# wangys16/FreeSplat

Measured on AMD Instinct MI355X. Metric: rendered views/sec @ 968x1296, 1.0M Gaussians, higher is better.
Workload: dtype f32

## Files before the change

freesplat_amd/csrc/raster_fwd.hip:

```cpp
#include <stdlib.h>

#include <type_traits>

#include "fs_common.h"

namespace fs {

template <int M>
__device__ __forceinline__ uint32_t lane_xor(uint32_t v)
{
    if constexpr (M == 1) return (uint32_t)__builtin_amdgcn_mov_dpp((int)v, 0xB1, 0xF, 0xF, true);
    else if constexpr (M == 2) return (uint32_t)__builtin_amdgcn_mov_dpp((int)v, 0x4E, 0xF, 0xF, true);
    else if constexpr (M == 3) return (uint32_t)__builtin_amdgcn_mov_dpp((int)v, 0x1B, 0xF, 0xF, true);
    else if constexpr (M < 32) return (uint32_t)__builtin_amdgcn_ds_swizzle((int)v, (M << 10) | 0x1F);
    else return (uint32_t)__shfl_xor((int)v, M, 64);
}
template <int M>
__device__ __forceinline__ unsigned long long lane_xor64(unsigned long long v)
{
    const uint32_t lo = lane_xor<M>((uint32_t)v), hi = lane_xor<M>((uint32_t)(v >> 32));
    return ((unsigned long long)hi << 32) | lo;
}

template <int DEG>
__device__ __forceinline__ void eval_sh(const float* __restrict__ sh, float3 dir, float* rgb,
                                        uint8_t& clampbits, int cs, int ks)
{
    float b[16];
    sh_basis<DEG>(dir.x, dir.y, dir.z, b);
    constexpr int NB = (DEG + 1) * (DEG + 1);
    clampbits = 0;
#pragma unroll
    for (int c = 0; c < 3; ++c) {
        const float* s = sh + c * cs;
        float acc = b[0] * s[0];
#pragma unroll
        for (int k = 1; k < NB; ++k) acc = acc + b[k] * s[k * ks];
        acc = acc + 0.5f;
        if (acc < 0.0f) clampbits |= (uint8_t)(1u << c);
        rgb[c] = fmaxf(acc, 0.0f);
    }
}

__device__ __forceinline__ void stage_rows(float* lds, const float* __restrict__ src, size_t base,
                                           int cnt, int per)
{
    const float* s = src + base * per;
    const int total = cnt * per;
    if ((((uintptr_t)s) & 15) == 0) {
        const int nv = total >> 2;
        int k = threadIdx.x;
        for (; k + 768 < nv; k += 1024) {
            const float4 v0 = ((const float4*)s)[k], v1 = ((const float4*)s)[k + 256];
            const float4 v2 = ((const float4*)s)[k + 512], v3 = ((const float4*)s)[k + 768];
            ((float4*)lds)[k] = v0; ((float4*)lds)[k + 256] = v1;
            ((float4*)lds)[k + 512] = v2; ((float4*)lds)[k + 768] = v3;
        }
        for (; k < nv; k += 256) ((float4*)lds)[k] = ((const float4*)s)[k];
        for (int k = (nv << 2) + threadIdx.x; k < total; k += blockDim.x) lds[k] = s[k];
    } else {
        for (int k = threadIdx.x; k < total; k += blockDim.x) lds[k] = s[k];
    }
}



struct QuadForm {
    float a, b, c;
    float Q;
    float D;
    float vplus;
    float Vmax;
    float inv2a;
};
__device__ __forceinline__ QuadForm quad_form(const float4 r0, const float4 r1)
{
    QuadForm f;
    f.a = -r0.z; f.c = -r0.w; f.b = -r1.x;
    f.Q = -(r1.z - 1e-3f * (1.0f + fabsf(r1.z)));
    f.D = 4.0f * f.a * f.c - f.b * f.b;
    const float invD = __builtin_amdgcn_rcpf(f.D);
    const float U = __builtin_amdgcn_sqrtf(fmaxf(4.0f * f.c * f.Q * invD, 0.0f));
    f.vplus = -f.b * __builtin_amdgcn_rcpf(2.0f * f.c) * U;
    f.Vmax = __builtin_amdgcn_sqrtf(fmaxf(4.0f * f.a * f.Q * invD, 0.0f));
    f.inv2a = __builtin_amdgcn_rcpf(2.0f * f.a);
    return f;
}
struct Band { float uL, uR; };
constexpr float kEps = 2e-5f;
__device__ __forceinline__ Band band_interval(const QuadForm& f, float vlo, float vhi)
{
    Band o;
    if (f.Q < 0.0f || vlo > f.Vmax + kEps || vhi < -f.Vmax - kEps) { o.uL = 3.0e38f; o.uR = -3.0e38f; return o; }
    const float vr = fminf(vhi, fmaxf(vlo, f.vplus)), vl = fminf(vhi, fmaxf(vlo, -f.vplus));
    const float sr = __builtin_amdgcn_sqrtf(fmaxf(4.0f * f.a * f.Q - f.D * vr * vr, 0.0f));
    const float sl = __builtin_amdgcn_sqrtf(fmaxf(4.0f * f.a * f.Q - f.D * vl * vl, 0.0f));
    o.uR = (-f.b * vr + sr) * f.inv2a;
    o.uL = (-f.b * vl - sl) * f.inv2a;
    const float w = kEps * (1.0f + fabsf(o.uR) + fabsf(o.uL));
    o.uR += w; o.uL -= w;
    return o;
}
struct RowBands { Band top, bot; };
__device__ __forceinline__ RowBands row_bands(const QuadForm& f, const float4 r0, int ty)
{
    const float v0 = (float)(ty * kTile) - r0.y;
    RowBands r;
    r.top = band_interval(f, v0, v0 + 7.0f);
    r.bot = band_interval(f, v0 + 8.0f, v0 + 15.0f);
    return r;
}
__device__ __forceinline__ uint32_t quad_mask_row(const RowBands& rb, const float4 r0, int tx)
{
    const float u0 = (float)(tx * kTile) - r0.x, u1 = u0 + 8.0f;
    uint32_t m = 0;
    if (!(u0 > rb.top.uR) && !(u0 + 7.0f < rb.top.uL)) m |= 1u;
    if (!(u1 > rb.top.uR) && !(u1 + 7.0f < rb.top.uL)) m |= 2u;
    if (!(u0 > rb.bot.uR) && !(u0 + 7.0f < rb.bot.uL)) m |= 4u;
    if (!(u1 > rb.bot.uR) && !(u1 + 7.0f < rb.bot.uL)) m |= 8u;
    return m;
}

__device__ __forceinline__ uint32_t band_cells(const Band& b, float px, int cell0, int ncell)
{
    const uint32_t full = ncell >= 32 ? 0xFFFFFFFFu : ((1u << ncell) - 1u);
    if (b.uL > b.uR) return 0u;
    if (!(b.uL <= b.uR)) return full;
    const float lo_f = ceilf((b.uL + px - 7.0f) * 0.125f - 1e-3f), hi_f = floorf((b.uR + px) * 0.125f + 1e-3f);
    const int lo = max((int)lo_f, cell0) - cell0, hi = min((int)hi_f, cell0 + ncell - 1) - cell0;
    if (lo > hi) return 0u;
    return ((2u << hi) - (1u << lo)) & full;
}
__device__ __forceinline__ unsigned long long pack_quad_masks(const QuadForm& f, const float4 r0, ushort4 rc)
{
    unsigned long long m = 0;
    const int rw = rc.z - rc.x, cell0 = 2 * rc.x, ncell = 2 * rw;
    int k = 0;
    for (int y = rc.y; y < rc.w; ++y) {
        const RowBands rb = row_bands(f, r0, y);
        const uint32_t top = band_cells(rb.top, r0.x, cell0, ncell), bot = band_cells(rb.bot, r0.x, cell0, ncell);
        for (int x = 0; x < rw; ++x, ++k) {
            const uint32_t nib = ((top >> (2 * x)) & 3u) | (((bot >> (2 * x)) & 3u) << 2);
            m |= (unsigned long long)nib << (4 * k);
        }
    }
    return m;
}

__device__ __forceinline__ uint32_t spread2(uint32_t x)
{
    x = (x | (x << 4)) & 0x0F0Fu;
    return (x | (x << 2)) & 0x3333u;
}
__device__ __forceinline__ unsigned long long pack_quad_masks4(const QuadForm& f, const float4 r0, ushort4 rc, bool cull, uint32_t& nz)
{
    unsigned long long m = 0;
    const int rw = rc.z - rc.x, rh = rc.w - rc.y, cell0 = 2 * rc.x, ncell = 2 * rw;
    const uint32_t rowfull = (1u << rw) - 1u;
    nz = 0u;
#pragma unroll
    for (int r = 0; r < 4; ++r) {
        if (r < rh) {
            const RowBands rb = row_bands(f, r0, rc.y + r);
            const uint32_t top = band_cells(rb.top, r0.x, cell0, ncell), bot = band_cells(rb.bot, r0.x, cell0, ncell);
            m |= (unsigned long long)(spread2(top) | (spread2(bot) << 2)) << (16 * r);
            uint32_t any = top | bot;
            any = (any | (any >> 1)) & 0x55u;
            any = (any | (any >> 1)) & 0x33u;
            any = (any | (any >> 2)) & 0x0Fu;
            nz |= (cull ? any : rowfull) << (4 * r);
        }
    }
    return m;
}

__device__ __forceinline__ void stage_rows_half(float* lds, const _Float16* __restrict__ src, size_t base, int cnt,
                                                int per)
{
    const _Float16* s = src + base * per;
    const int total = cnt * per;
    typedef _Float16 half8 __attribute__((ext_vector_type(8)));
    int done = 0;
    if ((((uintptr_t)s) & 15) == 0) {
        const int nv = total >> 3;
        auto put = [&](int k, const half8 v) {
            ((float4*)lds)[2 * k] = make_float4((float)v[0], (float)v[1], (float)v[2], (float)v[3]);
            ((float4*)lds)[2 * k + 1] = make_float4((float)v[4], (float)v[5], (float)v[6], (float)v[7]);
        };
        int k = threadIdx.x;
        for (; k + 256 < nv; k += 512) {
            const half8 v0 = ((const half8*)s)[k], v1 = ((const half8*)s)[k + 256];
            put(k, v0); put(k + 256, v1);
        }
        for (; k < nv; k += 256) put(k, ((const half8*)s)[k]);
        done = nv << 3;
    }
    for (int k = done + threadIdx.x; k < total; k += blockDim.x) lds[k] = (float)s[k];
}

struct Projected {
    float4 r0, r1, r2;
    ushort4 rect;
    uint8_t cb;
    int rad;
};
__device__ __forceinline__ Projected project_gaussian(
    const fs_raster_dims& d, bool live, float3 p_in, const float (&c_in)[6], float op, size_t i,
    const float* __restrict__ colors, const float* sh , int sh_cs, int sh_ks,
    const float* __restrict__ view, const float* __restrict__ proj, const float* __restrict__ campos,
    float tanfovx, float tanfovy, bool rescale, float wscale)
{
    Projected o;
    o.r0 = make_float4(0, 0, 0, 0); o.r1 = o.r0; o.r2 = o.r0;
    o.rect = make_ushort4(0, 0, 0, 0);
    o.cb = 0;
    o.rad = 0;
    float3 p = p_in;
    if (rescale) { p.x = p.x * wscale; p.y = p.y * wscale; p.z = p.z * wscale; }
    const float3 pv = xform43(view, p);
    if (live && pv.z > 0.2f) {
        const float4 ph = xform44(proj, p);
        const float pw = 1.0f / (ph.w + 0.0000001f);
        const float ndcx = ph.x * pw, ndcy = ph.y * pw;
        const float fx = (float)d.W / (2.0f * tanfovx), fy = (float)d.H / (2.0f * tanfovy);
        float c3[6];
#pragma unroll
        for (int k = 0; k < 6; ++k) c3[k] = c_in[k];
        if (rescale) {
            const float s2 = wscale * wscale;
#pragma unroll
            for (int k = 0; k < 6; ++k) c3[k] = c3[k] * s2;
        }
        const Cov2D cv = project_cov(view, p, c3, fx, fy, tanfovx, tanfovy);
        const float det = cv.a * cv.c - cv.b * cv.b;
        if (det != 0.0f) {
            const float det_inv = 1.0f / det;
            const float cA = cv.c * det_inv, cB = -cv.b * det_inv, cC = cv.a * det_inv;
            const float mid = 0.5f * (cv.a + cv.c);
            const float sq = sqrtf(fmaxf(0.1f, mid * mid - det));
            const float l1 = mid + sq, l2 = mid - sq;
            const float my_radius = ceilf(3.0f * sqrtf(fmaxf(l1, l2)));
            const float px = ((ndcx + 1.0f) * (float)d.W - 1.0f) * 0.5f;
            const float py = ((ndcy + 1.0f) * (float)d.H - 1.0f) * 0.5f;
            const int r = (int)my_radius;
            const int gx = (d.W + kTile - 1) / kTile, gy = (d.H + kTile - 1) / kTile;
            const int x0 = min(gx, max(0, (int)((px - (float)r) / (float)kTile)));
            const int y0 = min(gy, max(0, (int)((py - (float)r) / (float)kTile)));
            const int x1 = min(gx, max(0, (int)((px + (float)r + (float)(kTile - 1)) / (float)kTile)));
            const int y1 = min(gy, max(0, (int)((py + (float)r + (float)(kTile - 1)) / (float)kTile)));
            if ((x1 - x0) * (y1 - y0) > 0) {
                float rgb[3];
                if (colors) {
                    rgb[0] = colors[3 * i];
                    rgb[1] = colors[3 * i + 1];
                    rgb[2] = colors[3 * i + 2];
                } else {
                    float3 dir = make_float3(p.x - campos[0], p.y - campos[1], p.z - campos[2]);
                    const float len = sqrtf(dir.x * dir.x + dir.y * dir.y + dir.z * dir.z);
                    dir.x = dir.x / len; dir.y = dir.y / len; dir.z = dir.z / len;
                    switch (d.sh_degree) {
                        case 0: eval_sh<0>(sh, dir, rgb, o.cb, sh_cs, sh_ks); break;
                        case 1: eval_sh<1>(sh, dir, rgb, o.cb, sh_cs, sh_ks); break;
                        case 2: eval_sh<2>(sh, dir, rgb, o.cb, sh_cs, sh_ks); break;
                        default: eval_sh<3>(sh, dir, rgb, o.cb, sh_cs, sh_ks); break;
                    }
                }
                float thr;
                if (op > 0.0f) {
                    const float l = -logf(255.0f * op);
                    thr = l - (0.001f + 1e-5f * fabsf(l));
                } else {
                    thr = 1.0f;
                }
                o.r0 = make_float4(px, py, -0.5f * cA, -0.5f * cC);
                o.r1 = make_float4(-cB, op, thr, pv.z);
                o.r2 = make_float4(rgb[0], rgb[1], rgb[2], 0.0f);
                o.rect = make_ushort4((unsigned short)x0, (unsigned short)y0, (unsigned short)x1,
                                      (unsigned short)y1);
                o.rad = r;
            }
        }
    }
    return o;
}

template <bool SR>
__device__ __forceinline__ void load_mean_cov(const fs_raster_dims& d, const float* __restrict__ means3D,
                                              const float* __restrict__ cov3D, size_t i, float3& p_in, float (&c_in)[6])
{
    p_in = make_float3(means3D[3 * i], means3D[3 * i + 1], means3D[3 * i + 2]);
    if constexpr (SR) {
        float row[7];
#pragma unroll
        for (int k = 0; k < 7; ++k) row[k] = cov3D[7 * i + k];
        cov_from_scale_rot(row, c_in);
    } else if (d.flags & FS_RASTER_COV_FULL) {
        const float* cr = cov3D + 9 * i;
        c_in[0] = cr[0]; c_in[1] = cr[1]; c_in[2] = cr[2]; c_in[3] = cr[4]; c_in[4] = cr[5]; c_in[5] = cr[8];
    } else {
#pragma unroll
        for (int k = 0; k < 6; ++k) c_in[k] = cov3D[6 * i + k];
    }
}

constexpr int kWaveBins = 512;

__device__ __forceinline__ void bin_wave(const fs_raster_dims& d, int lane, uint32_t* s_cnt, uint32_t i, const Projected& pr,
                                         uint32_t* __restrict__ tile_counts, unsigned long long* __restrict__ keys,
                                         uint32_t tile_cap)
{
    const float4 r0 = pr.r0, r1 = pr.r1;
    const ushort4 rect = pr.rect;
    const bool valid = pr.rad > 0;
    const bool cull = (d.flags & FS_RASTER_TILE_CULL) != 0;
    const int gx = (d.W + kTile - 1) / kTile;
    const QuadForm qf = quad_form(r0, r1);
    const int rw = rect.z - rect.x, rh = rect.w - rect.y;
    const int area = rw * rh;
    const bool small = area <= 16;
    const bool all4 = __builtin_amdgcn_ballot_w64(valid && (rw > 4 || rh > 4)) == 0ull;
    unsigned long long qm = 0;
    uint32_t nz = 0u;
    if (all4) { if (valid) qm = pack_quad_masks4(qf, r0, rect, cull, nz); }
    else if (valid && small) qm = pack_quad_masks(qf, r0, rect);
    const unsigned long long key_hi = ((unsigned long long)__float_as_uint(r1.w) << 32) | (i << 4);
    int x0 = valid ? (int)rect.x : 0x7fff, y0 = valid ? (int)rect.y : 0x7fff;
    int x1 = valid ? (int)rect.z : 0, y1 = valid ? (int)rect.w : 0;
#define FS_BOX_STEP(M)                                                                                           \
    {                                                                                                            \
        const int lo = (int)lane_xor<M>((uint32_t)((x0 << 16) | y0)), hi = (int)lane_xor<M>((uint32_t)((x1 << 16) | y1)); \
        x0 = min(x0, lo >> 16); y0 = min(y0, lo & 0xffff);                                                       \
        x1 = max(x1, hi >> 16); y1 = max(y1, hi & 0xffff);                                                       \
    }
    FS_BOX_STEP(32) FS_BOX_STEP(16) FS_BOX_STEP(8) FS_BOX_STEP(4) FS_BOX_STEP(2) FS_BOX_STEP(1)
#undef FS_BOX_STEP
    const int bx0 = __builtin_amdgcn_readfirstlane(x0), by0 = __builtin_amdgcn_readfirstlane(y0);
    const int bw = max(0, __builtin_amdgcn_readfirstlane(x1) - bx0), bh = max(0, __builtin_amdgcn_readfirstlane(y1) - by0);
    const int nb = bw * bh;
    if (nb == 0) return;
    if (nb <= kWaveBins && all4) {
        for (int k = lane; k < nb; k += 64) s_cnt[k] = 0u;
        wave_lds_sync();
        const int cbase = (rect.y - by0) * bw + (rect.x - bx0);
        for (uint32_t z = nz; z != 0u; z &= z - 1u) {
            const int k = __builtin_ctz(z);
            atomicAdd(&s_cnt[cbase + (k >> 2) * bw + (k & 3)], 1u);
        }
        wave_lds_sync();
        for (int k0 = 0; k0 < nb; k0 += 64) {
            const int k = k0 + lane;
            if (k < nb) {
                const uint32_t c = s_cnt[k];
                const int ky = k / bw, kx = k - ky * bw;
                s_cnt[k] = c ? atomicAdd(&tile_counts[(by0 + ky) * gx + bx0 + kx], c) : 0u;
            }
        }
        wave_lds_sync();
        const uint32_t tbase = (uint32_t)(rect.y * gx + rect.x);
        for (uint32_t z = nz; z != 0u; z &= z - 1u) {
            const int k = __builtin_ctz(z);
            const uint32_t m = (uint32_t)(qm >> (4 * k)) & 15u;
            const uint32_t slot = atomicAdd(&s_cnt[cbase + (k >> 2) * bw + (k & 3)], 1u);
            if (slot < tile_cap) keys[(tbase + (uint32_t)((k >> 2) * gx + (k & 3))) * tile_cap + slot] = key_hi | m;
        }
        wave_lds_sync();
    } else if (nb <= kWaveBins) {
        for (int k = lane; k < nb; k += 64) s_cnt[k] = 0u;
        wave_lds_sync();
        if (valid) {
            int k = 0;
            for (int y = rect.y; y < rect.w; ++y) {
                RowBands rb = {};
                if (!small) rb = row_bands(qf, r0, y);
                for (int x = rect.x; x < rect.z; ++x, ++k) {
                    const uint32_t m = small ? (uint32_t)(qm >> (4 * k)) & 15u : quad_mask_row(rb, r0, x);
                    if (!cull || m) atomicAdd(&s_cnt[(y - by0) * bw + (x - bx0)], 1u);
                }
            }
        }
        wave_lds_sync();
        for (int k0 = 0; k0 < nb; k0 += 64) {
            const int k = k0 + lane;
            if (k < nb) {
                const uint32_t c = s_cnt[k];
                const int ky = k / bw, kx = k - ky * bw;
                s_cnt[k] = c ? atomicAdd(&tile_counts[(by0 + ky) * gx + bx0 + kx], c) : 0u;
            }
        }
        wave_lds_sync();
        if (valid) {
            int k = 0;
            for (int y = rect.y; y < rect.w; ++y) {
                RowBands rb = {};
                if (!small) rb = row_bands(qf, r0, y);
                for (int x = rect.x; x < rect.z; ++x, ++k) {
                    const uint32_t m = small ? (uint32_t)(qm >> (4 * k)) & 15u : quad_mask_row(rb, r0, x);
                    if (!cull || m) {
                        const uint32_t slot = atomicAdd(&s_cnt[(y - by0) * bw + (x - bx0)], 1u);
                        if (slot < tile_cap) keys[(uint32_t)(y * gx + x) * tile_cap + slot] = key_hi | m;
                    }
                }
            }
        }
        wave_lds_sync();
    } else if (all4) {
        const uint32_t tbase = (uint32_t)(rect.y * gx + rect.x);
        for (uint32_t z = nz; z != 0u; z &= z - 1u) {
            const int k = __builtin_ctz(z);
            const uint32_t m = (uint32_t)(qm >> (4 * k)) & 15u;
            const uint32_t tile = tbase + (uint32_t)((k >> 2) * gx + (k & 3));
            const uint32_t slot = atomicAdd(&tile_counts[tile], 1u);
            if (slot < tile_cap) keys[tile * tile_cap + slot] = key_hi | m;
        }
    } else if (valid) {
        int k = 0;
        for (int y = rect.y; y < rect.w; ++y) {
            RowBands rb = {};
            if (!small) rb = row_bands(qf, r0, y);
            for (int x = rect.x; x < rect.z; ++x, ++k) {
                const uint32_t m = small ? (uint32_t)(qm >> (4 * k)) & 15u : quad_mask_row(rb, r0, x);
                if (!cull || m) {
                    const uint32_t slot = atomicAdd(&tile_counts[y * gx + x], 1u);
                    if (slot < tile_cap) keys[(uint32_t)(y * gx + x) * tile_cap + slot] = key_hi | m;
                }
            }
        }
    }
}

__global__ __launch_bounds__(256) void zero_counts_kernel(char* base, size_t stride, int T)
{
    const int k = blockIdx.x * 256 + threadIdx.x;
    if (k < T) ((uint32_t*)(base + stride * blockIdx.y))[k] = 0u;
}

struct ViewBuffers {
    char* geom; size_t geom_stride;
    char* scratch; size_t scratch_stride;
    int32_t* radii;
};

#ifndef FS_PRE_WAVES
#define FS_PRE_WAVES 6
#endif
#define FS_PRE_OCC __attribute__((amdgpu_waves_per_eu(FS_PRE_WAVES, FS_PRE_WAVES)))
template <int CH, bool SR>
__global__ __launch_bounds__(256) FS_PRE_OCC void preprocess_views_kernel(
    fs_raster_dims d, int v, const float* __restrict__ means3D, const float* __restrict__ cov3D,
    const float* __restrict__ shs, const float* __restrict__ colors, const float* __restrict__ opacities,
    const float* __restrict__ view, const float* __restrict__ proj, const float* __restrict__ campos,
    const float* __restrict__ tanfov_dev, const float* __restrict__ scale_dev, ViewBuffers vb, uint32_t tile_cap)
{
    extern __shared__ __attribute__((aligned(16))) float lds[];
    constexpr int kPerBlock = 64 * CH;
    const int base = blockIdx.x * kPerBlock;
    const int cnt = min(kPerBlock, d.N - base);
    const int per_sh = shs ? d.M * 3 : 0;
    const bool sh_cm = (d.flags & FS_RASTER_SH_CHANNEL_MAJOR) != 0;
    const int sh_cs = sh_cm ? d.M : 1, sh_ks = sh_cm ? 1 : 3;
    float* const l_sh = lds;
    if (shs) {
        if (d.flags & FS_RASTER_SH_FP16) stage_rows_half(l_sh, (const _Float16*)shs, base, cnt, per_sh);
        else stage_rows(l_sh, shs, base, cnt, per_sh);
    }
    const int t = threadIdx.x, lane = t & 63, wave = t >> 6;
    const int chunk = wave % CH;
    uint32_t* const s_cnt_base = (uint32_t*)(lds + (size_t)kPerBlock * per_sh);
    uint32_t* const s_cnt = s_cnt_base + wave * kWaveBins;
    const int li = chunk * 64 + lane;
    const bool live = li < cnt;
    const uint32_t i = (uint32_t)(base + li);
    float* const l_g = (float*)(s_cnt_base + 4 * kWaveBins) + li;
    {
        float3 p_in = make_float3(0.0f, 0.0f, 0.0f);
        float c_in[6] = {0, 0, 0, 0, 0, 0};
        float op = 0.0f;
        if (live) {
            load_mean_cov<SR>(d, means3D, cov3D, i, p_in, c_in);
            op = opacities[i];
        }
        if (wave < CH) {
            l_g[0 * kPerBlock] = p_in.x; l_g[1 * kPerBlock] = p_in.y; l_g[2 * kPerBlock] = p_in.z;
#pragma unroll
            for (int k = 0; k < 6; ++k) l_g[(3 + k) * kPerBlock] = c_in[k];
            l_g[9 * kPerBlock] = op;
        }
    }
    __syncthreads();
    const int T = num_tiles(d.H, d.W);
    const size_t keys_off = align_up((size_t)T * 4, 256);
#pragma nounroll
    for (int j0 = wave / CH; j0 < v; j0 += 4 / CH) {
        const int j = __builtin_amdgcn_readfirstlane(j0);
        int li_ = li, lane_ = lane;
        asm volatile("" : "+v"(li_), "+v"(lane_));
        const float* const lg = (const float*)(s_cnt_base + 4 * kWaveBins) + li_;
        const float3 p_in = make_float3(lg[0 * kPerBlock], lg[1 * kPerBlock], lg[2 * kPerBlock]);
        float c_in[6];
#pragma unroll
        for (int k = 0; k < 6; ++k) c_in[k] = lg[(3 + k) * kPerBlock];
        const float op = lg[9 * kPerBlock];
        const float tanfovx = tanfov_dev ? tanfov_dev[2 * j] : d.tanfovx;
        const float tanfovy = tanfov_dev ? tanfov_dev[2 * j + 1] : d.tanfovy;
        const float wscale = scale_dev ? scale_dev[j] : 1.0f;
        const Projected pr = project_gaussian(d, live, p_in, c_in, op, i, colors, l_sh + (size_t)li_ * per_sh, sh_cs, sh_ks,
                                              view + 16 * j, proj + 16 * j, campos + 3 * j, tanfovx, tanfovy,
                                              scale_dev != nullptr, wscale);
        if (live) {
            const GeomView g = geom_view(vb.geom + vb.geom_stride * j, d.N);
            g.rec[3 * (size_t)i + 0] = pr.r0;
            g.rec[3 * (size_t)i + 1] = pr.r1;
            g.rec[3 * (size_t)i + 2] = pr.r2;
            if (!(d.flags & FS_RASTER_NO_BACKWARD_STATE)) {
                g.rect[i] = pr.rect;
                g.clamp[i] = pr.cb;
            }
            if (vb.radii) vb.radii[(size_t)j * d.N + i] = pr.rad;
        }
        char* const sc = vb.scratch + vb.scratch_stride * j;
        bin_wave(d, lane_, s_cnt, i, pr, (uint32_t*)sc, (unsigned long long*)(sc + keys_off), tile_cap);
    }
}

__global__ __launch_bounds__(1024) void tile_scan_kernel(const char* __restrict__ counts0, size_t counts_stride,
                                                         char* __restrict__ offsets0, size_t offsets_stride, int T,
                                                         uint32_t* __restrict__ counters0,
                                                         unsigned long long cap, uint32_t tile_cap)
{
    const uint32_t* __restrict__ counts = (const uint32_t*)(counts0 + counts_stride * blockIdx.x);
    uint32_t* __restrict__ offsets = (uint32_t*)(offsets0 + offsets_stride * blockIdx.x);
    uint32_t* __restrict__ counters = counters0 + 2 * blockIdx.x;
    __shared__ uint32_t s_wave[16];
    __shared__ uint32_t s_max[16];
    __shared__ unsigned long long s_wide[16];
    const int t = threadIdx.x, lane = t & 63, wave = t >> 6;
    const int per = (T + 1023) / 1024;
    const int lo = min(T, t * per), hi = min(T, lo + per);
    uint32_t s = 0, mx = 0;
    unsigned long long wide = 0;
    for (int k = lo; k < hi; ++k) { const uint32_t c = counts[k]; s += c; wide += c; mx = max(mx, c); }
#pragma unroll
    for (int d = 32; d >= 1; d >>= 1) {
        wide += __shfl_xor(wide, d, 64);
        mx = max(mx, (uint32_t)__shfl_xor((int)mx, d, 64));
    }
    if (lane == 0) { s_wide[wave] = wide; s_max[wave] = mx; }
    uint32_t inc = s;
#pragma unroll
    for (int d = 1; d < 64; d <<= 1) {
        const uint32_t o = __shfl_up(inc, d, 64);
        if (lane >= d) inc += o;
    }
    if (lane == 63) s_wave[wave] = inc;
    __syncthreads();
    uint32_t before = 0, total = 0;
#pragma unroll
    for (int k = 0; k < 16; ++k) {
        const uint32_t v = s_wave[k];
        before += k < wave ? v : 0u;
        total += v;
    }
    inc += before;
    uint32_t run = inc - s;
    for (int k = lo; k < hi; ++k) {
        offsets[k] = run;
        run += counts[k];
    }
    if (t == 1023) {
        unsigned long long total64 = 0;
        uint32_t maxc = 0;
#pragma unroll
        for (int k = 0; k < 16; ++k) { total64 += s_wide[k]; maxc = max(maxc, s_max[k]); }
        offsets[T] = total;
        counters[0] = total64 > 0xFFFFFFFFull ? 0xFFFFFFFFu : (uint32_t)total64;
        counters[1] = (total64 > cap || maxc > tile_cap) ? max(maxc, 1u) : 0u;
    }
}

#ifndef FS_SORT_LDS
#define FS_SORT_LDS 1792
#endif
constexpr int kSortLds = FS_SORT_LDS;

template <typename Ptr>
__device__ __forceinline__ void bitonic_sort_any(Ptr a, uint32_t n)
{
    uint32_t P = 1;
    while (P < n) P <<= 1;
    const uint32_t half = P >> 1;
    for (uint32_t k = 2; k <= P; k <<= 1) {
        const uint32_t hk = k >> 1;
        for (uint32_t t = threadIdx.x; t < half; t += blockDim.x) {
            const uint32_t blk = t / hk, off = t % hk;
            const uint32_t i = blk * k + off, j = blk * k + (k - 1 - off);
            if (j < n) {
                const unsigned long long x = a[i], y = a[j];
                if (x > y) { a[i] = y; a[j] = x; }
            }
        }
        __syncthreads();
        for (uint32_t s = k >> 2; s >= 1; s >>= 1) {
            for (uint32_t t = threadIdx.x; t < half; t += blockDim.x) {
                const uint32_t i = (t / s) * 2 * s + (t % s), j = i + s;
                if (j < n) {
                    const unsigned long long x = a[i], y = a[j];
                    if (x > y) { a[i] = y; a[j] = x; }
                }
            }
            __syncthreads();
        }
    }
}

template <int EPT, int TM, bool REV>
__device__ __forceinline__ void thread_exchange(unsigned long long (&k)[EPT], int t, unsigned long long* lds)
{
    constexpr int HB = TM >= 128 ? 128 : TM >= 64 ? 64 : TM >= 32 ? 32 : TM >= 16 ? 16 : TM >= 8 ? 8 : TM >= 4 ? 4 : TM >= 2 ? 2 : 1;
    const bool low = (t & HB) == 0;
    unsigned long long y[EPT];
    if constexpr (TM < 64) {
#pragma unroll
        for (int e = 0; e < EPT; ++e) y[e] = lane_xor64<TM>(k[REV ? EPT - 1 - e : e]);
    } else {
        constexpr int CH = EPT * 256 > kSortLds ? kSortLds / 256 : EPT;
#pragma unroll
        for (int e0 = 0; e0 < EPT; e0 += CH) {
            __syncthreads();
#pragma unroll
            for (int e = 0; e < CH; ++e) lds[e * 256 + t] = k[REV ? EPT - 1 - (e0 + e) : e0 + e];
            __syncthreads();
#pragma unroll
            for (int e = 0; e < CH; ++e) y[e0 + e] = lds[e * 256 + (t ^ TM)];
        }
    }
#pragma unroll
    for (int e = 0; e < EPT; ++e) {
        const unsigned long long x = k[e];
        k[e] = low ? (y[e] < x ? y[e] : x) : (y[e] > x ? y[e] : x);
    }
}

template <int EPT, int J>
struct Clean {
    static __device__ __forceinline__ void run(unsigned long long (&k)[EPT], int t, unsigned long long* lds)
    {
        if constexpr (J >= EPT) {
            thread_exchange<EPT, J / EPT, false>(k, t, lds);
        } else {
#pragma unroll
            for (int e = 0; e < EPT; ++e)
                if ((e & J) == 0) {
                    const unsigned long long a = k[e], b = k[e | J];
                    if (a > b) { k[e] = b; k[e | J] = a; }
                }
        }
        if constexpr (J > 1) Clean<EPT, J / 2>::run(k, t, lds);
    }
};
template <int EPT, int K>
struct Stages {
    static __device__ __forceinline__ void run(unsigned long long (&k)[EPT], int t, unsigned long long* lds)
    {
        if constexpr (K > 2) Stages<EPT, K / 2>::run(k, t, lds);
        if constexpr (K <= EPT) {
#pragma unroll
            for (int e = 0; e < EPT; ++e) {
                const int p = e ^ (K - 1);
                if (e < p) {
                    const unsigned long long a = k[e], b = k[p];
                    if (a > b) { k[e] = b; k[p] = a; }
                }
            }
        } else {
            thread_exchange<EPT, K / EPT - 1, true>(k, t, lds);
        }
        if constexpr (K >= 4) Clean<EPT, K / 4>::run(k, t, lds);
    }
};

constexpr uint32_t kMaxBucket = 24;
template <int EPT>
__device__ __forceinline__ void sort_tile_buckets(const unsigned long long* keys, uint32_t* __restrict__ gout,
                                                  uint32_t n, unsigned long long* sk, uint32_t* cnt, uint32_t* s_red,
                                                  int tid = -1)
{
    constexpr int CAP = 256 * EPT;
    uint32_t* const list = cnt;
    const int t = tid >= 0 ? tid : (int)threadIdx.x, lane = t & 63, wave = t >> 6;
    unsigned long long k[EPT];
    uint32_t zmin = 0xFFFFFFFFu, zmax = 0u;
#pragma unroll
    for (int e = 0; e < EPT; ++e) {
        const uint32_t i = (uint32_t)(e * 256 + t);
        k[e] = i < n ? keys[i] : ~0ull;
        cnt[i] = 0u;
        if (i < n) {
            const uint32_t z = (uint32_t)(k[e] >> 32);
            zmin = min(zmin, z);
            zmax = max(zmax, z);
        }
    }
    if (t == 0) cnt[CAP] = 0u;
#pragma unroll
    for (int m = 32; m >= 1; m >>= 1) {
        zmin = min(zmin, (uint32_t)__shfl_xor((int)zmin, m, 64));
        zmax = max(zmax, (uint32_t)__shfl_xor((int)zmax, m, 64));
    }
    if (lane == 0) { s_red[wave] = zmin; s_red[4 + wave] = zmax; }
    __syncthreads();
    zmin = min(min(s_red[0], s_red[1]), min(s_red[2], s_red[3]));
    zmax = max(max(s_red[4], s_red[5]), max(s_red[6], s_red[7]));
    const float scale = (float)CAP / (float)(zmax - zmin + 1u);
// ... 709 lines not shown
```

Measured before the change: 4757.

## Streamline quad-mask packing and wave binning with compact masks and ISA intrinsics

Replaces the 64-bit per-quad nibble mask in the 4x4 binning path with two 32-bit top/bottom cell masks built by a new row_cells8 routine. That routine computes band intervals with med3/bfm instructions instead of row_bands plus band_cells plus bit spreading. The wave bounding-box reduction now uses packed 16-bit min/max, the tile division by box width uses a float reciprocal, and the 16-slot loops iterate with a scalar bit test instead of ctz over a divergent mask. The aim is fewer VALU instructions and less divergence in the binning kernel; the float-reciprocal division and the reimplemented interval math risk off-by-one differences at edges.

Result: no change. 4797, median of 6 (+0.9%).

```diff
diff --git a/freesplat_amd/csrc/raster_fwd.hip b/freesplat_amd/csrc/raster_fwd.hip
--- a/freesplat_amd/csrc/raster_fwd.hip
+++ b/freesplat_amd/csrc/raster_fwd.hip
@@ -147,31 +147,78 @@
     return m;
 }
 
-__device__ __forceinline__ uint32_t spread2(uint32_t x)
-{
-    x = (x | (x << 4)) & 0x0F0Fu;
-    return (x | (x << 2)) & 0x3333u;
-}
-__device__ __forceinline__ unsigned long long pack_quad_masks4(const QuadForm& f, const float4 r0, ushort4 rc, bool cull, uint32_t& nz)
-{
-    unsigned long long m = 0;
-    const int rw = rc.z - rc.x, rh = rc.w - rc.y, cell0 = 2 * rc.x, ncell = 2 * rw;
-    const uint32_t rowfull = (1u << rw) - 1u;
-    nz = 0u;
+struct QuadMasks4 { uint32_t top, bot; };
+__device__ __forceinline__ uint32_t quad_nibble(const QuadMasks4& q, int k)
+{
+    return __builtin_amdgcn_ubfe(q.top, 2 * k, 2) | (__builtin_amdgcn_ubfe(q.bot, 2 * k, 2) << 2);
+}
+struct RowConsts {
+    float aQ4, nb, vtop, vbot;
+    int cell0, cellN;
+    uint32_t full;
+    bool none;
+};
+__device__ __forceinline__ int med3i(int x, int lo, int hi)
+{
+    int r;
+    asm("v_med3_i32 %0, %1, %2, %3" : "=v"(r) : "v"(x), "v"(lo), "v"(hi));
+    return r;
+}
+__device__ __forceinline__ uint32_t bit_field_mask(int width, int first)
+{
+    uint32_t r;
+    asm("v_bfm_b32 %0, %1, %2" : "=v"(r) : "v"(width), "v"(first));
+    return r;
+}
+__device__ __forceinline__ void row_cells8(const QuadForm& f, const RowConsts& k, const float4 r0, int ty, uint32_t& top, uint32_t& bot)
+{
+    const float v0 = (float)(ty * kTile) - r0.y;
+    const float vlo[2] = {v0, v0 + 8.0f}, vhi[2] = {v0 + 7.0f, v0 + 15.0f};
+    uint32_t m[2];
+#pragma unroll
+    for (int h = 0; h < 2; ++h) {
+        const float vr = fminf(vhi[h], fmaxf(vlo[h], f.vplus)), vl = fminf(vhi[h], fmaxf(vlo[h], -f.vplus));
+        const float sr = __builtin_amdgcn_sqrtf(fmaxf(k.aQ4 - f.D * vr * vr, 0.0f));
+        const float sl = __builtin_amdgcn_sqrtf(fmaxf(k.aQ4 - f.D * vl * vl, 0.0f));
+        float uR = (k.nb * vr + sr) * f.inv2a, uL = (k.nb * vl - sl) * f.inv2a;
+        const float w = kEps * (1.0f + fabsf(uR) + fabsf(uL));
+        uR += w; uL -= w;
+        const float lo_f = (uL + r0.x - 7.0f) * 0.125f - 1e-3f, hi_f = (uR + r0.x) * 0.125f + 1e-3f;
+        const int lo = med3i((int)ceilf(lo_f), k.cell0, k.cellN);
+        const int lo1 = lo - 1, hi = med3i((int)floorf(hi_f), lo1, k.cellN - 1);
+        const uint32_t cells = bit_field_mask(hi - lo1, lo - k.cell0);
+        const bool empty = k.none || vlo[h] > k.vtop || vhi[h] < k.vbot;
+        m[h] = (!empty && uL <= uR) ? cells : ((empty || uL > uR) ? 0u : k.full);
+    }
+    top = m[0]; bot = m[1];
+}
+__device__ __forceinline__ QuadMasks4 pack_quad_masks4(const QuadForm& f, const float4 r0, ushort4 rc, bool cull, uint32_t& nz)
+{
+    QuadMasks4 q = {0u, 0u};
+    const int rw = rc.z - rc.x, rh = rc.w - rc.y;
+    RowConsts k;
+    k.aQ4 = 4.0f * f.a * f.Q; k.nb = -f.b; k.vtop = f.Vmax + kEps; k.vbot = -f.Vmax - kEps;
+    k.cell0 = 2 * rc.x; k.cellN = k.cell0 + 2 * rw; k.full = (1u << (2 * rw)) - 1u; k.none = f.Q < 0.0f;
 #pragma unroll
     for (int r = 0; r < 4; ++r) {
         if (r < rh) {
-            const RowBands rb = row_bands(f, r0, rc.y + r);
-            const uint32_t top = band_cells(rb.top, r0.x, cell0, ncell), bot = band_cells(rb.bot, r0.x, cell0, ncell);
-            m |= (unsigned long long)(spread2(top) | (spread2(bot) << 2)) << (16 * r);
-            uint32_t any = top | bot;
-            any = (any | (any >> 1)) & 0x55u;
-            any = (any | (any >> 1)) & 0x33u;
-            any = (any | (any >> 2)) & 0x0Fu;
-            nz |= (cull ? any : rowfull) << (4 * r);
-        }
-    }
-    return m;
+            uint32_t top, bot;
+            row_cells8(f, k, r0, rc.y + r, top, bot);
+            q.top |= top << (8 * r);
+            q.bot |= bot << (8 * r);
+        }
+    }
+    if (cull) {
+        uint32_t any = q.top | q.bot;
+        any = (any | (any >> 1)) & 0x55555555u;
+        any = (any | (any >> 1)) & 0x33333333u;
+        any = (any | (any >> 2)) & 0x0F0F0F0Fu;
+        any = (any | (any >> 4)) & 0x00FF00FFu;
+        nz = (any | (any >> 8)) & 0xFFFFu;
+    } else {
+        nz = (0x1111u * ((1u << rw) - 1u)) & ((1u << (4 * rh)) - 1u);
+    }
+    return q;
 }
 
 __device__ __forceinline__ void stage_rows_half(float* lds, const _Float16* __restrict__ src, size_t base, int cnt,
@@ -305,6 +352,17 @@
 
 constexpr int kWaveBins = 512;
 
+__device__ __forceinline__ uint32_t slot_bit(int k)
+{
+    uint32_t b = 1u << k;
+    asm("" : "+s"(b));
+    return b;
+}
+__device__ __forceinline__ int box_row(int k, float inv_bw)
+{
+    return (int)(((float)k + 0.5f) * inv_bw);
+}
+
 __device__ __forceinline__ void bin_wave(const fs_raster_dims& d, int lane, uint32_t* s_cnt, uint32_t i, const Projected& pr,
                                          uint32_t* __restrict__ tile_counts, unsigned long long* __restrict__ keys,
                                          uint32_t tile_cap)
@@ -320,48 +378,56 @@
     const bool small = area <= 16;
     const bool all4 = __builtin_amdgcn_ballot_w64(valid && (rw > 4 || rh > 4)) == 0ull;
     unsigned long long qm = 0;
+    QuadMasks4 q4 = {0u, 0u};
     uint32_t nz = 0u;
-    if (all4) { if (valid) qm = pack_quad_masks4(qf, r0, rect, cull, nz); }
+    if (all4) { if (valid) q4 = pack_quad_masks4(qf, r0, rect, cull, nz); }
     else if (valid && small) qm = pack_quad_masks(qf, r0, rect);
     const unsigned long long key_hi = ((unsigned long long)__float_as_uint(r1.w) << 32) | (i << 4);
-    int x0 = valid ? (int)rect.x : 0x7fff, y0 = valid ? (int)rect.y : 0x7fff;
-    int x1 = valid ? (int)rect.z : 0, y1 = valid ? (int)rect.w : 0;
+    typedef unsigned short u16x2 __attribute__((ext_vector_type(2)));
+    u16x2 lo2 = valid ? (u16x2){rect.y, rect.x} : (u16x2){0x7fff, 0x7fff};
+    u16x2 hi2 = valid ? (u16x2){rect.w, rect.z} : (u16x2){0, 0};
 #define FS_BOX_STEP(M)                                                                                           \
     {                                                                                                            \
-        const int lo = (int)lane_xor<M>((uint32_t)((x0 << 16) | y0)), hi = (int)lane_xor<M>((uint32_t)((x1 << 16) | y1)); \
-        x0 = min(x0, lo >> 16); y0 = min(y0, lo & 0xffff);                                                       \
-        x1 = max(x1, hi >> 16); y1 = max(y1, hi & 0xffff);                                                       \
+        lo2 = __builtin_elementwise_min(lo2, __builtin_bit_cast(u16x2, lane_xor<M>(__builtin_bit_cast(uint32_t, lo2)))); \
+        hi2 = __builtin_elementwise_max(hi2, __builtin_bit_cast(u16x2, lane_xor<M>(__builtin_bit_cast(uint32_t, hi2)))); \
     }
     FS_BOX_STEP(32) FS_BOX_STEP(16) FS_BOX_STEP(8) FS_BOX_STEP(4) FS_BOX_STEP(2) FS_BOX_STEP(1)
 #undef FS_BOX_STEP
-    const int bx0 = __builtin_amdgcn_readfirstlane(x0), by0 = __builtin_amdgcn_readfirstlane(y0);
-    const int bw = max(0, __builtin_amdgcn_readfirstlane(x1) - bx0), bh = max(0, __builtin_amdgcn_readfirstlane(y1) - by0);
+    const uint32_t blo = (uint32_t)__builtin_amdgcn_readfirstlane((int)__builtin_bit_cast(uint32_t, lo2));
+    const uint32_t bhi = (uint32_t)__builtin_amdgcn_readfirstlane((int)__builtin_bit_cast(uint32_t, hi2));
+    const int bx0 = (int)(blo >> 16), by0 = (int)(blo & 0xffffu);
+    const int bw = max(0, (int)(bhi >> 16) - bx0), bh = max(0, (int)(bhi & 0xffffu) - by0);
     const int nb = bw * bh;
     if (nb == 0) return;
+    const float inv_bw = __builtin_amdgcn_rcpf((float)bw);
     if (nb <= kWaveBins && all4) {
         for (int k = lane; k < nb; k += 64) s_cnt[k] = 0u;
         wave_lds_sync();
         const int cbase = (rect.y - by0) * bw + (rect.x - bx0);
-        for (uint32_t z = nz; z != 0u; z &= z - 1u) {
-            const int k = __builtin_ctz(z);
-            atomicAdd(&s_cnt[cbase + (k >> 2) * bw + (k & 3)], 1u);
+#pragma nounroll
+        for (int k = 0; k < 16; ++k) {
+            if (nz & slot_bit(k)) atomicAdd(&s_cnt[cbase + ((k >> 2) * bw + (k & 3))], 1u);
         }
         wave_lds_sync();
         for (int k0 = 0; k0 < nb; k0 += 64) {
             const int k = k0 + lane;
             if (k < nb) {
                 const uint32_t c = s_cnt[k];
-                const int ky = k / bw, kx = k - ky * bw;
+                const int ky = box_row(k, inv_bw), kx = k - ky * bw;
                 s_cnt[k] = c ? atomicAdd(&tile_counts[(by0 + ky) * gx + bx0 + kx], c) : 0u;
             }
         }
         wave_lds_sync();
         const uint32_t tbase = (uint32_t)(rect.y * gx + rect.x);
-        for (uint32_t z = nz; z != 0u; z &= z - 1u) {
-            const int k = __builtin_ctz(z);
-            const uint32_t m = (uint32_t)(qm >> (4 * k)) & 15u;
-            const uint32_t slot = atomicAdd(&s_cnt[cbase + (k >> 2) * bw + (k & 3)], 1u);
-            if (slot < tile_cap) keys[(tbase + (uint32_t)((k >> 2) * gx + (k & 3))) * tile_cap + slot] = key_hi | m;
+        uint32_t kbase = tbase * tile_cap;
+        asm("" : "+v"(kbase));
+#pragma nounroll
+        for (int k = 0; k < 16; ++k) {
+            if (nz & slot_bit(k)) {
+                const uint32_t m = quad_nibble(q4, k);
+                const uint32_t slot = atomicAdd(&s_cnt[cbase + ((k >> 2) * bw + (k & 3))], 1u);
+                if (slot < tile_cap) keys[kbase + (uint32_t)((k >> 2) * gx + (k & 3)) * tile_cap + slot] = key_hi | m;
+            }
         }
         wave_lds_sync();
     } else if (nb <= kWaveBins) {
@@ -383,7 +449,7 @@
             const int k = k0 + lane;
             if (k < nb) {
                 const uint32_t c = s_cnt[k];
-                const int ky = k / bw, kx = k - ky * bw;
+                const int ky = box_row(k, inv_bw), kx = k - ky * bw;
                 s_cnt[k] = c ? atomicAdd(&tile_counts[(by0 + ky) * gx + bx0 + kx], c) : 0u;
             }
         }
@@ -407,7 +473,7 @@
         const uint32_t tbase = (uint32_t)(rect.y * gx + rect.x);
         for (uint32_t z = nz; z != 0u; z &= z - 1u) {
             const int k = __builtin_ctz(z);
-            const uint32_t m = (uint32_t)(qm >> (4 * k)) & 15u;
+            const uint32_t m = quad_nibble(q4, k);
             const uint32_t tile = tbase + (uint32_t)((k >> 2) * gx + (k & 3));
             const uint32_t slot = atomicAdd(&tile_counts[tile], 1u);
             if (slot < tile_cap) keys[tile * tile_cap + slot] = key_hi | m;
```
